# LJacksonPan/RaTrack

Hardware: AMD Instinct MI355X
Metric: radar frame-pairs/sec (backbone forward, eval) at B=64,N=256 per GPU (higher is better)
Workload: dtype f32 (2xfp16 split MFMA: three fp16 products per fp32 product, fp32 accumulate, power-of-two scales per matrix and position); 1 GPU; Track4D.backbone forward, B=64 frame-pairs x N=256 points per GPU, S=512 centroids, eval-mode BN, random-init weights, hipGraph=True, batches in flight=4; global_batch=64, parallelism=replicas x1 (no collective on the forward path)

## Files before the change

### include/rtk_fused.h

```cpp
#ifndef RTK_FUSED_H
#define RTK_FUSED_H

#include "rtk_pointnet2.h"

#ifdef __cplusplus
extern "C" {
#endif

#define RTK_MAX_SRC 4
#define RTK_MAX_LAYERS 4

typedef struct {
    const float *ptr;
    int pitch;
    int channels;
    int per_sample;
} rtk_src_t;

#define RTK_LAYER_SPLIT 0x100
typedef struct {
    const float *w_packed;
    const float *bias;
    int cin16, cout16;
    int act;
// ... 55 lines not shown
                                     int out_pitch, int out_channel_major, rtk_stream_t stream);

RTK_EXPORT int rtk_pack_split_layer(int cout, int cin, const float *w, int transposed, void *image, float *inv_scale,
                                    rtk_stream_t stream);
RTK_EXPORT int rtk_cost_volume_split(int samples, int n1, int n2, const float *xyz1, const float *xyz2,
                                     const int64_t *knn_idx, const float *p1, const float *p2, const float *wd_packed,
                                     const void *split_images, const float *image_scales, const float *bias2,
                                     const float *bias3, const rtk_layer_t *wn, float *out, int out_pitch, rtk_stream_t stream);
RTK_EXPORT int rtk_cost_volume_split_shared(int samples, int n1, int n2, const float *xyz1, const float *xyz2,
                                            const int64_t *knn_idx, const float *p1, const float *p2, const float *wd_packed,
                                            const void *split_images, const float *image_scales, const float *bias2,
                                            const float *bias3, const rtk_layer_t *wn, float *out, int out_pitch, int workgroups,
                                            rtk_stream_t stream);
RTK_EXPORT int rtk_cost_volume_split_gconst(int samples, int n1, int n2, const float *xyz1, const float *xyz2,
                                            const int64_t *knn_idx, const float *p1, const float *p2, const float *wd_packed,
                                            const void *split_images, const float *image_scales, const float *bias2,
                                            const float *bias3, const rtk_layer_t *wn, float *out, int out_pitch, int workgroups,
                                            rtk_stream_t stream);
RTK_EXPORT int rtk_cost_volume_split_term(int samples, int n1, int n2, const float *xyz1, const float *xyz2,
                                          const int64_t *knn_idx, const float *p1, const float *p2, const float *sample_term,
                                          const float *wd_packed, const void *split_images, const float *image_scales,
                                          const float *bias2, const float *bias3, const rtk_layer_t *wn, float *out, int out_pitch,
                                          int workgroups, rtk_stream_t stream);
RTK_EXPORT int rtk_sa_scale_split(int samples, int n, int npoint, int nsample, const float *xyz, const float *new_xyz,
                                  const int *idx, const float *q, int q_pitch, int c1, const float *w1xyz_packed,
                                  const void *split_image, const float *image_scale, const float *bias2, float *out, int out_pitch,
                                  int out_offset, const int *src_nuniq, const int *dst_nuniq, rtk_stream_t stream);
RTK_EXPORT int rtk_sa_scale_split_serial(int samples, int n, int npoint, int nsample, const float *xyz, const float *new_xyz,
                                         const int *idx, const float *q, int q_pitch, int c1, const float *w1xyz_packed,
                                         const void *split_image, const float *image_scale, const float *bias2, float *out,
                                         int out_pitch, int out_offset, const int *src_nuniq, const int *dst_nuniq,
                                         rtk_stream_t stream);
RTK_EXPORT int rtk_split_mlp2(int positions, const float *x, const void *images, const float *image_scales, const float *bias1,
                              const float *bias2, float *y, rtk_stream_t stream);

RTK_EXPORT int rtk_prepare_inputs(int b, int n, const float *pc1, const float *pc2, const float *feature1,
                                  const float *feature2, float *xyz, float *raw, rtk_stream_t stream);

RTK_EXPORT int rtk_fps_centroids(int b, int n, int npoint, const float *xyz, int *idx, float *new_xyz, int *nuniq,
                                 int *tie, const int *n_valid, float *snap, int *first_tie, rtk_stream_t stream);

RTK_EXPORT int rtk_knn_point_masked(int b, int s, int n, int k, const float *query, const float *points, int64_t *idx,
                                    const int *n_valid, rtk_stream_t stream);

RTK_EXPORT int rtk_fps_relevel(int b, int npoint, int levels, const float *xyz1, const int *nuniq1, const int *tie,
                               int *idx, float *new_xyz, int *nuniq, int *tie_work, const int *idx1, const float *snap1,
// ... 115 lines not shown
```

### ratrack_amd/abi.py

```python
import ctypes

import torch

_i, _l, _f, _d, _p = ctypes.c_int, ctypes.c_long, ctypes.c_float, ctypes.c_double, ctypes.c_void_p
_ip, _fp, _pp, P = ctypes.POINTER(_i), ctypes.POINTER(_f), ctypes.POINTER(_p), ctypes.POINTER



class Src(ctypes.Structure):
    _fields_ = [("ptr", _p), ("pitch", _i), ("channels", _i), ("per_sample", _i)]


class Layer(ctypes.Structure):
    _fields_ = [("w_packed", _p), ("bias", _p), ("cin16", _i), ("cout16", _i), ("act", _i), ("inv_scale", _f)]


class Interp(ctypes.Structure):
    _fields_ = [("known_feats", _p), ("pitch", _i), ("channels", _i), ("m", _i), ("idx", _p), ("dist2", _p), ("nuniq", _p)]


class GtermJob(ctypes.Structure):
    _fields_ = [("wt", _p), ("bias", _p), ("out", _p), ("cout", _i), ("s0", _i), ("count", _i), ("out_pitch", _i), ("wt2", _p), ("s2", _i)]


# ... 122 lines not shown
    "rtk_group_points_grad": [_i] * 5 + [_p] * 3 + [_p],
    "rtk_group_points_grad_set": [_i] * 5 + [_p] * 3 + [_p],
    "rtk_three_nn": [_i] * 3 + [_p] * 4 + [_p],
    "rtk_knn": [_i] * 4 + [_p] * 4 + [_p],
    "rtk_three_interpolate": [_i] * 4 + [_p] * 4 + [_p],
    "rtk_three_interpolate_grad": [_i] * 4 + [_p] * 4 + [_p],
    "rtk_three_interpolate_grad_set": [_i] * 4 + [_p] * 4 + [_p],
    "rtk_knn_point": [_i] * 4 + [_p] * 3 + [_p],
    "rtk_pointwise_mlp": [_i, _i, P(Interp), _i, P(Src), _p, _i, P(Layer), _p, _i, _i, _i, _p, _p, _p],
    "rtk_pointwise_mlp_pipelined": [_i, _i, P(Interp), _i, P(Src), _p, _i, P(Layer), _p, _i, _i, _i, _p, _p, _p],
    "rtk_pointwise_mlp_tap": [_i, _i, P(Interp), P(Layer), _p, _i, _p, P(Layer), _i, _p, _i, _p],
    "rtk_pointwise_mlp_tap_pipelined": [_i, _i, P(Interp), P(Layer), _p, _i, _p, P(Layer), _i, _p, _i, _p],
    "rtk_pointwise_mlp_pair": [_i, _i, _i, P(Src), _p, P(Layer), _p, _i, _i, _i, P(Layer), _p, _i, _p],
    "rtk_sa_scale": [_i] * 4 + [_p] * 4 + [_i, _i, _p, _i, P(Layer), _p, _i, _i, _p, _p, _p],
    "rtk_sa_scale_serial": [_i] * 4 + [_p] * 4 + [_i, _i, _p, _i, P(Layer), _p, _i, _i, _p, _p, _p],
    "rtk_cost_volume": [_i] * 3 + [_p] * 6 + [P(Layer), P(Layer), _p, _i, _p],
    "rtk_patch_cost": [_i] * 2 + [_p] * 3 + [_i, P(Layer), _p, _i, _i, _p],
    "rtk_patch_cost_wave16": [_i] * 2 + [_p] * 3 + [_i, P(Layer), _p, _i, _i, _p],
    "rtk_pack_split_layer": [_i, _i, _p, _i, _p, _p, _p],
    "rtk_cost_volume_split": [_i] * 3 + [_p] * 10 + [P(Layer), _p, _i, _p],
    "rtk_cost_volume_split_shared": [_i] * 3 + [_p] * 10 + [P(Layer), _p, _i, _i, _p],
    "rtk_cost_volume_split_gconst": [_i] * 3 + [_p] * 10 + [P(Layer), _p, _i, _i, _p],
    "rtk_cost_volume_split_term": [_i] * 3 + [_p] * 11 + [P(Layer), _p, _i, _i, _p],
    "rtk_sa_scale_split": [_i] * 4 + [_p] * 4 + [_i, _i, _p, _p, _p, _p, _p, _i, _i, _p, _p, _p],
    "rtk_sa_scale_split_serial": [_i] * 4 + [_p] * 4 + [_i, _i, _p, _p, _p, _p, _p, _i, _i, _p, _p, _p],
    "rtk_split_mlp2": [_i, _p, _p, _p, _p, _p, _p, _p],
    "rtk_prepare_inputs": [_i] * 2 + [_p] * 6 + [_p],
    "rtk_fps_centroids": [_i] * 3 + [_p] * 8 + [_p],
    "rtk_knn_point_masked": [_i] * 4 + [_p] * 4 + [_p],
    "rtk_fps_relevel": [_i] * 3 + [_p] * 9 + [_i, _p, _p],
    "rtk_gru_step": [_i] * 3 + [_p] * 8 + [_p],
    "rtk_gru_step_head": [_i] * 3 + [_p] * 11 + [_i, _p],
    "rtk_global_terms": [_i, _i, _p, _i, P(GtermJob), _p, _i, _i, _p],
    "rtk_copy_multi": [_i, P(CopyJob), _p],
    "rtk_to_channel_major": [_i] * 3 + [_p, _i, _i, _p, _i, _i, _p],
    "rtk_ball_query_pair": [_i] * 3 + [_f, _i, _f, _i] + [_p] * 5 + [_p],
    "rtk_three_nn_masked": [_i] * 3 + [_p] * 6 + [_p],
    "rtk_geometry_front": [_i] * 4 + [_p, _p, _i] + [_p] * 13 + [_p, _p, _i, _p],
    "rtk_geometry_tables": [_i] * 3 + [_p] * 3 + [_fp, _ip, _pp, _pp, _pp, _p],
    "rtk_to_channel_major_multi": [_i] * 3 + [_p, _p],
    "rtk_log_sinkhorn": [_i, _i, _p, _f, _i, _p, _p],
    "rtk_dbscan": [_i, _p, _i, _p, _p, _f, _d, _i, _p, _p],
    "rtk_dbscan_batched": [_p, _f, _d, _i, _i, _p, _p, _p, _p, _p, _l, _p],
    "rtk_object_descriptors": [_p, _i, _p, _p, _p, _p, _p, _p],
    "rtk_affinity_pairs": [_i, _i] + [_p] * 7 + [_p],
    "rtk_associate_batched": [_i] * 3 + [_p] * 7 + [_f, _i] + [_p] * 9 + [_p],
# ... 99 lines not shown
```

### ratrack_amd/csrc/fused_split.hip

```cpp
#include "rtk_common.h"
#include "rtk_fused.h"
#include "split_mfma.h"

namespace {

#ifndef SP_NW
#define SP_NW 4
#endif
#ifndef SP_F
#define SP_F 32
#endif
constexpr int CV_F = 32;

__global__ __launch_bounds__(256) void pack_split_kernel(int cout, int cin, const float *__restrict__ w, int transposed, u4v *__restrict__ out,
                                                         float *__restrict__ inv_scale) {
    __shared__ unsigned s_m[4];
    float m = 0.f;
    const f4 *w4 = reinterpret_cast<const f4 *>(w);
    for (int i = threadIdx.x; i < cout * cin / 4; i += 256) {
        const f4 t = w4[i];
        m = __builtin_fmaxf(__builtin_fmaxf(m, __builtin_fabsf(t.x)), __builtin_fabsf(t.y));
        m = __builtin_fmaxf(__builtin_fmaxf(m, __builtin_fabsf(t.z)), __builtin_fabsf(t.w));
    }
    unsigned mb = __float_as_uint(m);
#pragma unroll
    for (int d = 32; d >= 1; d >>= 1) { const unsigned o = __shfl_xor(mb, d, 64); mb = o > mb ? o : mb; }
    if ((threadIdx.x & 63) == 0) s_m[threadIdx.x >> 6] = mb;
    __syncthreads();
    mb = max(max(s_m[0], s_m[1]), max(s_m[2], s_m[3]));
    const LaneScale sc = lane_scale_of(mb);
    if (blockIdx.x == 0 && threadIdx.x == 0) *inv_scale = sc.inv;
    const int VB = cout / 32, slot = blockIdx.x * 256 + threadIdx.x;
    if (slot >= (cin / 16) * VB * 64) return;
    const int lane = slot & 63, v = (slot >> 6) % VB, s = (slot >> 6) / VB, hh = lane >> 5, i = lane & 31;
    const int o = 32 * v + i, c0 = 32 * (s >> 1) + 16 * (s & 1) + 4 * hh;
    f4 x0, x1;
    if (transposed) {
#pragma unroll
        for (int r = 0; r < 4; ++r) { x0[r] = w[(size_t)(c0 + r) * cout + o]; x1[r] = w[(size_t)(c0 + 8 + r) * cout + o]; }
    } else {
        const float *row = w + (size_t)o * cin + c0;
        x0 = *reinterpret_cast<const f4 *>(row); x1 = *reinterpret_cast<const f4 *>(row + 8);
    }
    u4v b[2];
    split2(x0, x1, sc.s, b);
#pragma unroll
    for (int p = 0; p < 2; ++p) out[((size_t)(s * VB + v) * 2 + p) * 64 + lane] = b[p];
}

__device__ __forceinline__ f4 leaky_med4(f4 t, float inf) {
    const f4 u = t * 0.1f;
    return (f4){__builtin_amdgcn_fmed3f(t.x, u.x, inf), __builtin_amdgcn_fmed3f(t.y, u.y, inf), __builtin_amdgcn_fmed3f(t.z, u.z, inf),
                __builtin_amdgcn_fmed3f(t.w, u.w, inf)};
}
__device__ __forceinline__ f4 scale_bias4(f4 a, float c, f4 b) { return __builtin_elementwise_fma(a, (f4){c, c, c, c}, b); }

__global__ __launch_bounds__(64 * SP_NW) __attribute__((amdgpu_waves_per_eu(1, 1)))
void split_mlp2_kernel(int positions, const float *__restrict__ x, const f4 *__restrict__ blob, const float *__restrict__ wsc,
                       const float *__restrict__ bias1, const float *__restrict__ bias2, float *__restrict__ y) {
    const float kinf = rtk_hidden_inf();
    __shared__ __attribute__((aligned(16))) f4 s_w[2 * SP_F * 64];
    const int lane = threadIdx.x & 63, wave = __builtin_amdgcn_readfirstlane(threadIdx.x >> 6), hh = lane >> 5, col = lane & 31;
    constexpr int NF = 2 * SPLIT_NF;
    WStreamA<SP_NW, SP_F, NF> ws;
    ws.start_parts(blob, s_w, wave, lane);
// ... 408 lines not shown
                for (int e = 0; e < 4; ++e) r[q][e] = relu1(w[4 * q + e], kinf) * h[4 * v + q][e];
            const f4 t = row_sum16_transpose4(r[0], r[1], r[2], r[3]);
            if (valid && (j & 3) == 0) *reinterpret_cast<f4 *>(o + 32 * v + 8 * (2 * ((j >> 3) & 1) + ((j >> 2) & 1))) = t;
        };
        out_block(0);
        out_block(1);
        float cn[6] = {0.f, 0.f, 0.f, 0.f, 0.f, 0.f};
        f4 q0n = q0, q1n = q1, s0n = q0, s1n = q1;
        if (more) {
#pragma unroll
            for (int c = 0; c < 3; ++c) { cn[c] = ldc(P.xyz2 + nbn * 3 + c); cn[3 + c] = ldc(P.xyz1 + in_ * 3 + c); }
            q0n = ldc4(P.p1 + in_ * 256 + 4 * hh + 8 * j); q1n = ldc4(P.p1 + in_ * 256 + 4 * hh + 8 * (16 + j));
        }
        if (more && P.st) { s0n = ldc4(P.st + bn * 256 + 4 * hh + 8 * j); s1n = ldc4(P.st + bn * 256 + 4 * hh + 8 * (16 + j)); }
#pragma unroll
        for (int v = 2; v < SPLIT_VB; ++v) out_block(v);
        pt = ptn; valid = validn; i = in_; nb = nbn; q0 = q0n; q1 = q1n;
        if (P.st) { q0 = add4_rn(q0n, s0n); q1 = add4_rn(q1n, s1n); }
        dx = __fsub_rn(cn[0], cn[3]); dy = __fsub_rn(cn[1], cn[4]); dz = __fsub_rn(cn[2], cn[5]);
    }
    ws.finish();
}

struct CvSplitBwdParams {
    CvSplitParams f;
    const float *dout;
    int dout_pitch;
    const float *a3;
    const uint2 *mk1, *mk2;
    float *dz1, *dz2, *dz3, *dq3, *d4, *dp1, *dpd, *dt2, *dbrows;
};

__device__ __forceinline__ f4 leaky_grad_bits4(f4 d, unsigned bits) {
    return (f4){(bits & 1u) ? d.x : 0.1f * d.x, (bits & 2u) ? d.y : 0.1f * d.y, (bits & 4u) ? d.z : 0.1f * d.z, (bits & 8u) ? d.w : 0.1f * d.w};
}

__global__ __launch_bounds__(64 * SP_NW) __attribute__((amdgpu_waves_per_eu(1, 1))) void cost_volume_bwd_split_kernel(const CvSplitBwdParams Q) {
    const float kinf = rtk_hidden_inf();
    __shared__ __attribute__((aligned(16))) f4 s_w[2 * SP_F * 64];
    __shared__ float s_wct[128 * 64];
    const CvSplitParams &P = Q.f;
    const int lane = threadIdx.x & 63, wave = __builtin_amdgcn_readfirstlane(threadIdx.x >> 6), hh = lane >> 5, col = lane & 31, pp = col >> 4,
              j = col & 15;
    const int jq = 2 * ((j >> 3) & 1) + ((j >> 2) & 1);
    for (int e = threadIdx.x; e < 128 * 64; e += 64 * SP_NW) {
        const int l = e & 63, st = e >> 6, o = l & 31, ch = 32 * (st >> 4) + 8 * ((st >> 2) & 3) + 4 * (l >> 5) + (st & 3);
// ... 478 lines not shown
        float *o = P.out + (long)c * P.out_pitch + P.out_offset + 4 * hh + 8 * qo;
        if constexpr (NS == 32) {
            f4 t[4];
#pragma unroll
            for (int q = 0; q < 4; ++q) t[q] = wave_max_pair16(m[0][q], m[1][q], kinf);
            const f4 r = relu_med4(row_max16_transpose4(t[0], t[1], t[2], t[3]), kinf);
            if (valid && (col & 3) == 0) *reinterpret_cast<f4 *>(o + 32 * ((col >> 4) & 1)) = r;
        } else {
#pragma unroll
            for (int v = 0; v < 2; ++v) {
                const f4 r = relu_med4(row_max16_transpose4(m[v][0], m[v][1], m[v][2], m[v][3]), kinf);
                if (valid && (col & 3) == 0) *reinterpret_cast<f4 *>(o + 32 * v) = r;
            }
        }
    }
}

}

extern "C" int rtk_pack_split_layer(int cout, int cin, const float *w, int transposed, void *image, float *inv_scale, rtk_stream_t stream) {
    RTK_REQUIRE(cout > 0 && cin > 0 && cout % 32 == 0 && cin % 32 == 0 && w && image && inv_scale, "pack_split_layer: bad arguments");
    RTK_REQUIRE((long)cout * cin <= (1L << 22), "pack_split_layer: more than 2^22 weights (every workgroup scans the matrix for its scale)");
    const int slots = (cin / 16) * (cout / 32) * 64;
    pack_split_kernel<<<(slots + 255) / 256, 256, 0, (hipStream_t)stream>>>(cout, cin, w, transposed, (u4v *)image, inv_scale);
    RTK_CHECK_LAUNCH("pack_split_layer");
    return RTK_OK;
}

extern "C" int rtk_split_mlp2(int positions, const float *x, const void *images, const float *image_scales, const float *bias1,
                              const float *bias2, float *y, rtk_stream_t stream) {
    RTK_REQUIRE(positions > 0 && x && images && image_scales && bias1 && bias2 && y, "split_mlp2: bad arguments");
    const int tiles = (positions + 32 * SP_NW - 1) / (32 * SP_NW);
    split_mlp2_kernel<<<tiles < 256 ? tiles : 256, 64 * SP_NW, 0, (hipStream_t)stream>>>(positions, x, (const f4 *)images, image_scales, bias1, bias2, y);
    RTK_CHECK_LAUNCH("split_mlp2");
    return RTK_OK;
}

static int cv_split_fill(const char *who, CvSplitParams &P, int samples, int n1, int n2, const float *xyz1, const float *xyz2,
                         const int64_t *knn_idx, const void *split_images, const float *image_scales, const rtk_layer_t *wn, dim3 &grid) {
    RTK_REQUIRE(samples > 0 && samples <= 65535 && n1 > 0 && n2 >= 16 && xyz1 && xyz2 && knn_idx && split_images && image_scales,
                "%s: bad arguments", who);
    RTK_REQUIRE(wn && wn[0].w_packed && wn[1].w_packed && wn[2].w_packed && wn[1].bias && wn[2].bias && wn[1].cin16 == 1 &&
                wn[1].cout16 == 1 && wn[2].cin16 == 1 && wn[2].cout16 == 16, "%s: bad WeightNet layers", who);
    P.samples = samples; P.n1 = n1; P.n2 = n2;
    P.xyz1 = xyz1; P.xyz2 = xyz2; P.knn = knn_idx;
    P.blob = reinterpret_cast<const f4 *>(split_images);
    P.wsc = image_scales;
    P.wn.wa = wn[0].w_packed; P.wn.wb = wn[1].w_packed; P.wn.wc = wn[2].w_packed; P.wn.bb = wn[1].bias; P.wn.bc = wn[2].bias;
    P.p1 = P.p2 = P.st = P.wd = P.bias2 = P.bias3 = nullptr;
    P.out = nullptr; P.out_pitch = 0; P.sv1 = P.sv2 = P.sv3 = nullptr; P.mk1 = P.mk2 = nullptr; P.amax = nullptr;
    const int groups = (n1 + 2 * SP_NW - 1) / (2 * SP_NW);
    int gx = 256 / samples;
    if (gx < 1) gx = 1;
    if (gx > groups) gx = groups;
    grid = rtk_xcd_grid(samples, gx, P.gx);
    return RTK_OK;
}

static int cu_count() {
    int dev = 0, n = 0;
    if (hipGetDevice(&dev) != hipSuccess || hipDeviceGetAttribute(&n, hipDeviceAttributeMultiprocessorCount, dev) != hipSuccess || n < 8) return 256;
    return n;
}

static int cv_split_forward(const char *who, int samples, int n1, int n2, const float *xyz1, const float *xyz2, const int64_t *knn_idx,
                            const float *p1, const float *p2, const float *wd_packed, const void *split_images, const float *image_scales,
                            const float *bias2, const float *bias3, const rtk_layer_t *wn, float *out, int out_pitch, float *a1, float *a2,
                            float *a3, void *mask1, void *mask2, float *amax, int workgroups, rtk_stream_t stream,
                            const float *sample_term = nullptr, bool global_consts = false) {
    CvSplitParams P;
    dim3 grid;
    if (cv_split_fill(who, P, samples, n1, n2, xyz1, xyz2, knn_idx, split_images, image_scales, wn, grid) != RTK_OK) return RTK_ERR_INVALID;
    RTK_REQUIRE(p1 && p2 && wd_packed && bias2 && bias3 && out, "%s: bad arguments", who);
    RTK_REQUIRE((double)samples * n2 <= 4194304.0, "%s: more than 2^22 rows in p2 (32-bit byte offsets of the row requests): split the batch", who);
    RTK_REQUIRE(out_pitch % 4 == 0 && out_pitch >= 256, "%s: bad out_pitch", who);
    const bool save = a1 != nullptr;
    RTK_REQUIRE(!save || ((double)samples * n1 * 16.0 * 1024.0 < 4294967296.0), "%s: more than 4 GiB per saved activation (32-bit row "
                "offsets): split the batch", who);
    P.p1 = p1; P.p2 = p2; P.st = sample_term; P.wd = wd_packed; P.bias2 = bias2; P.bias3 = bias3; P.out = out; P.out_pitch = out_pitch;
    P.sv1 = a1; P.sv2 = a2; P.sv3 = a3; P.mk1 = (uint2 *)mask1; P.mk2 = (uint2 *)mask2; P.amax = amax;
    if (samples % 8 == 0) {
        const int tiles_x = (samples / 8) * ((n1 + 2 * SP_NW - 1) / (2 * SP_NW));
        int per_xcd = (workgroups > 0 ? workgroups : cu_count()) / 8;
        if (per_xcd < 1) per_xcd = 1;
        if (per_xcd > tiles_x) per_xcd = tiles_x;
        P.gx = 8 * per_xcd;
        grid = dim3(P.gx);
    }
    if (save) cost_volume_split_kernel<true><<<grid, 64 * SP_NW, 0, (hipStream_t)stream>>>(P);
    else if (global_consts) cost_volume_split_kernel<false, false><<<grid, 64 * SP_NW, 0, (hipStream_t)stream>>>(P);
    else cost_volume_split_kernel<false><<<grid, 64 * SP_NW, 0, (hipStream_t)stream>>>(P);
    RTK_CHECK_LAUNCH(who);
    return RTK_OK;
}

extern "C" int rtk_cost_volume_split(int samples, int n1, int n2, const float *xyz1, const float *xyz2, const int64_t *knn_idx,
                                     const float *p1, const float *p2, const float *wd_packed, const void *split_images,
                                     const float *image_scales, const float *bias2, const float *bias3, const rtk_layer_t *wn, float *out,
                                     int out_pitch, rtk_stream_t stream) {
    return cv_split_forward("cost_volume_split", samples, n1, n2, xyz1, xyz2, knn_idx, p1, p2, wd_packed, split_images, image_scales, bias2, bias3,
                            wn, out, out_pitch, nullptr, nullptr, nullptr, nullptr, nullptr, nullptr, 0, stream);
}

extern "C" int rtk_cost_volume_split_shared(int samples, int n1, int n2, const float *xyz1, const float *xyz2, const int64_t *knn_idx,
                                            const float *p1, const float *p2, const float *wd_packed, const void *split_images,
                                            const float *image_scales, const float *bias2, const float *bias3, const rtk_layer_t *wn,
                                            float *out, int out_pitch, int workgroups, rtk_stream_t stream) {
    RTK_REQUIRE(workgroups >= 0, "cost_volume_split_shared: workgroups = %d", workgroups);
    return cv_split_forward("cost_volume_split_shared", samples, n1, n2, xyz1, xyz2, knn_idx, p1, p2, wd_packed, split_images, image_scales,
                            bias2, bias3, wn, out, out_pitch, nullptr, nullptr, nullptr, nullptr, nullptr, nullptr, workgroups, stream);
}

extern "C" int rtk_cost_volume_split_gconst(int samples, int n1, int n2, const float *xyz1, const float *xyz2, const int64_t *knn_idx,
                                            const float *p1, const float *p2, const float *wd_packed, const void *split_images,
                                            const float *image_scales, const float *bias2, const float *bias3, const rtk_layer_t *wn,
                                            float *out, int out_pitch, int workgroups, rtk_stream_t stream) {
    RTK_REQUIRE(workgroups >= 0, "cost_volume_split_gconst: workgroups = %d", workgroups);
    return cv_split_forward("cost_volume_split_gconst", samples, n1, n2, xyz1, xyz2, knn_idx, p1, p2, wd_packed, split_images, image_scales,
                            bias2, bias3, wn, out, out_pitch, nullptr, nullptr, nullptr, nullptr, nullptr, nullptr, workgroups, stream, nullptr, true);
}

extern "C" int rtk_cost_volume_split_term(int samples, int n1, int n2, const float *xyz1, const float *xyz2, const int64_t *knn_idx,
                                          const float *p1, const float *p2, const float *sample_term, const float *wd_packed,
                                          const void *split_images, const float *image_scales, const float *bias2, const float *bias3,
                                          const rtk_layer_t *wn, float *out, int out_pitch, int workgroups, rtk_stream_t stream) {
    RTK_REQUIRE(workgroups >= 0 && sample_term, "cost_volume_split_term: workgroups = %d, sample_term = %p", workgroups, (const void *)sample_term);
    return cv_split_forward("cost_volume_split_term", samples, n1, n2, xyz1, xyz2, knn_idx, p1, p2, wd_packed, split_images, image_scales,
                            bias2, bias3, wn, out, out_pitch, nullptr, nullptr, nullptr, nullptr, nullptr, nullptr, workgroups, stream, sample_term);
}

extern "C" int rtk_cost_volume_split_train(int samples, int n1, int n2, const float *xyz1, const float *xyz2, const int64_t *knn_idx,
                                           const float *p1, const float *p2, const float *wd_packed, const void *split_images,
                                           const float *image_scales, const float *bias2, const float *bias3, const rtk_layer_t *wn,
                                           float *out, int out_pitch, float *a1, float *a2, float *a3, void *mask1, void *mask2,
                                           float *act_amax, rtk_stream_t stream) {
    RTK_REQUIRE(a1 && a2 && a3 && mask1 && mask2, "cost_volume_split_train: null activation buffer");
    return cv_split_forward("cost_volume_split_train", samples, n1, n2, xyz1, xyz2, knn_idx, p1, p2, wd_packed, split_images, image_scales,
                            bias2, bias3, wn, out, out_pitch, a1, a2, a3, mask1, mask2, act_amax, 0, stream);
}

extern "C" int rtk_cost_volume_bwd_split(int samples, int n1, int n2, const float *xyz1, const float *xyz2, const int64_t *knn_idx,
                                         const void *split_images_t, const float *image_scales_t, const rtk_layer_t *wn, const float *dout,
                                         int dout_pitch,
                                         const float *a3, const void *mask1, const void *mask2, float *dz1, float *dz2, float *dz3,
                                         float *dq3, float *d4, float *dp1, float *dpd, float *dt2, float *dbias_rows,
                                         float *dz_amax, rtk_stream_t stream) {
    CvSplitBwdParams Q;
    dim3 grid;
    if (cv_split_fill("cost_volume_bwd_split", Q.f, samples, n1, n2, xyz1, xyz2, knn_idx, split_images_t, image_scales_t, wn, grid) != RTK_OK)
        return RTK_ERR_INVALID;
    RTK_REQUIRE(dout && mask1 && mask2 && a3 && dz1 && dz2 && dz3 && dq3 && d4 && dp1 && dpd && dt2, "cost_volume_bwd_split: bad arguments");
// ... 64 lines not shown
```

### ratrack_amd/fused.py

```python
import ctypes
import os
import types

import torch

from . import _lib
from . import pointnet2_hip as _native
from .abi import CopyJob as _CopyJob, GtermJob as _GtJob, Interp as _Interp, Layer as _Layer, Src as _Src, ptr as _ptr, stream as _stream

ACT_NONE, ACT_RELU, ACT_LEAKY, ACT_SIGMOID = 0, 1, 2, 3


def copy_multi(pairs):
    for i in range(0, len(pairs), 8):
        part = pairs[i:i + 8]
        jobs = (_CopyJob * len(part))()
        for j, (d, s_) in enumerate(part):
            assert d.is_contiguous() and s_.is_contiguous() and d.shape == s_.shape and d.dtype == s_.dtype and d.device == s_.device
            jobs[j].src, jobs[j].dst, jobs[j].bytes = s_.data_ptr(), d.data_ptr(), d.numel() * d.element_size()
        _lib.call("rtk_copy_multi", len(part), jobs, _stream())


def ceil16(c):
    return (c + 15) // 16 * 16
# ... 497 lines not shown
        if self.side is not None:
            ev = torch.cuda.Event()
            ev.record(self.side)
            self.events[key] = ev

    def wait(self, key):
        ev = self.events.get(key)
        if ev is not None:
            torch.cuda.current_stream().wait_event(ev)

    def head(self, count):
        g = object.__new__(Geometry)
        g.n, g.samples, g.npoint = self.n, count, self.npoint
        g.xyz = [x[:count] for x in self.xyz]
        g.ball = [[b[:count] for b in row] for row in self.ball]
        g.nuniq = [c[:count] for c in self.nuniq]
        g.fps_idx, g.tie = [i[:count] for i in self.fps_idx], self.tie[:count]
        g.events, g.knn, g.side = self.events, self.knn, self.side
        g.nn = {k: (d2[:count], idx[:count], m) for k, (d2, idx, m) in self.nn.items()}
        return g


CV_SPLIT_MAX_ROWS = 1 << 22


def cv_shared_workgroups(samples, n1, dev):
    cus = torch.cuda.get_device_properties(dev).multi_processor_count
    if samples % 8 or cus % 8:
        return 0
    tiles = (samples // 8) * ((n1 + 7) // 8)
    lo, hi = max(1, cus // 16), max(1, cus // 8 * 3 // 4)
    balance = lambda w: tiles / (w * -(-tiles // w))
    ok = [w for w in range(hi, lo - 1, -1) if balance(w) >= 0.95]
    w = ok[0] if ok else max(range(lo, hi + 1), key=balance)
    return 8 * min(w, tiles)


SA_ENTRIES = ("rtk_sa_scale", "rtk_sa_scale_split")
SA_ENTRIES_SERIAL = ("rtk_sa_scale_serial", "rtk_sa_scale_split_serial")


def sa_scale(geo, W, lvl, s, q, qcol, out, out_offset):
    sc = W.scales[lvl][s]
    qptr, qpitch = _colptr(q, qcol)
    optr, opitch = _colptr(out)
    src, dst = geo.xyz[lvl], geo.xyz[lvl + 1]
# ... 75 lines not shown
        self.enc = _PNHeadWeights(sd, "pn_head.", dev)
        self.dec = _PNHeadWeights(sd, "fd_layer.mse.", dev)
        z = lambda n: torch.zeros(n, dtype=torch.float64, device=sd["bin_score"].device)
        self.enc_q1 = Chain([(self.enc.wq1, z(32), ACT_NONE)], dev)
        self.enc_q1_w = self.enc.wq1.float().to(dev).contiguous()
        w0 = sd["fc_layer.mlp_convs.0.weight"].double().reshape(256, 515)
        b0 = sd["fc_layer.mlp_convs.0.bias"].double()
        self.p1_loc = Chain([(w0[:, 0:128], z(256), ACT_NONE)], dev)
        self.p2_loc = Chain([(w0[:, 256:384], z(256), ACT_NONE)], dev)
        tr = lambda w: w.float().t().contiguous().to(dev)
        self.p1_glob_wt, self.p1_glob_b = tr(w0[:, 128:256]), b0.float().to(dev).contiguous()
        self.p2_glob_wt = tr(w0[:, 384:512])
        self.cv_wd = offset_image(torch.cat([w0[:, 512:515], z(256)[:, None]], 1), dev)
        self.cv_layers = Chain([(sd["fc_layer.mlp_convs.%d.weight" % i].double().reshape(256, 256),
                                 sd["fc_layer.mlp_convs.%d.bias" % i].double(), ACT_LEAKY) for i in (1, 2)], dev)
        self.cv_split = bool(split)
        w23 = [sd["fc_layer.mlp_convs.%d.weight" % i].double().reshape(256, 256).float().to(dev).contiguous() for i in (1, 2)]
        self.cv_bias23 = torch.stack([sd["fc_layer.mlp_convs.%d.bias" % i].double().float() for i in (1, 2)]).to(dev).contiguous()
        self.cv_images = torch.empty(2 * SPLIT_IMAGE_256, dtype=torch.int16, device=dev)
        self.cv_scales = torch.empty(2, dtype=torch.float32, device=dev)
        for l, w in enumerate(w23):
            _lib.call("rtk_pack_split_layer", 256, 256, w.data_ptr(), 0, self.cv_images[l * SPLIT_IMAGE_256:].data_ptr(),
                      self.cv_scales[l:].data_ptr(), _stream())
        torch.cuda.current_stream().synchronize()
        self.wn1 = _WeightNet(sd, "fc_layer.weightnet1", dev)
        self.wn2 = _WeightNet(sd, "fc_layer.weightnet2", dev)
        def predictor(prefix, first_cols):
            layers = []
            for i in range(3):
                w, b = fold_bn(sd["%s.sf_mlp.%d.0.weight" % (prefix, i)], "%s.sf_mlp.%d.1" % (prefix, i), sd)
                layers.append([w, b, ACT_RELU])
            return layers
        cp = predictor("fd_layer.cp", None)
        wl, bl = sd["fd_layer.cp.linear.weight"].double(), sd["fd_layer.cp.linear.bias"].double()
        wc2 = sd["fd_layer.cp.conv2.weight"].double().reshape(3, 32)
        cp.append([wl @ wc2, bl, ACT_SIGMOID])
        self.cls_head = Chain([tuple(x) for x in cp], dev)
        fp = predictor("fd_layer.fp", None)
        w_first = fp[0][0]
        self.flow_glob_wt, self.flow_glob_b = tr(w_first[:, 128:256]), fp[0][1].float().to(dev).contiguous()
        fp[0] = [w_first[:, 0:128], z(128), ACT_RELU]
        fp.append([sd["fd_layer.fp.conv2.weight"].double().reshape(3, 32), z(3), ACT_NONE])
        self.flow_head = Chain([tuple(x) for x in fp], dev)
        wq = self.dec.wq1
        wq_pad = torch.zeros(32, 16, dtype=torch.float64, device=wq.device)
        wq_pad[:, :2] = wq[:, 0:2]
# ... 70 lines not shown
            q1d = pointwise(B * N, N, dsrc, self.dec_q1, new(B * N, 32), sample_bias=sbq)
        prop, gfeat = run_pnhead(self.dec, geo.head(B), q1d, gmax=gmax[2 * B:])
        if h is None:
            h = torch.zeros(5, B, 128, device=dev, dtype=torch.float32)
        gout, h_out, sbf = self._gru_step(gfeat, h)
        flow = torch.empty(B, 3, N, dtype=torch.float32, device=dev)
        pointwise(B * N, N, [(prop, 128, False)], self.flow_head, flow, out_channels=3, sample_bias=sbf, channel_major=True)
        f12 = feat12.view(2 * B, N, 256).permute(0, 2, 1)
        pc1_features, pc2_features = f12[:B], f12[B:]
        cor_cm = cor.view(B, N, 256).permute(0, 2, 1)
        prop_cm = prop.view(B, N, 128).permute(0, 2, 1)
        return flow, h_out, cls, cor_cm, pc1_features, pc2_features, prop_cm

    def _cost_volume(self, B, N, x1, x2, knn1, p1, p2, cor1, sample_term=None):
        assert sample_term is None or self.cv_split
        if _TRACE is not None:
            _TRACE.append(("cost_volume", B * N * 16, 3 * 256 + 2 * 256 * 256 + (3 * 8 + 8 * 8 + 8 * 256) + 256))
        if self.cv_split:
            step = B if B * N <= CV_SPLIT_MAX_ROWS else max(1, CV_SPLIT_MAX_ROWS // N)
            for b0 in range(0, B, step):
                nb = min(step, B - b0)
                wgs = cv_shared_workgroups(nb, N, x1.device) if self.cv_shared else 0
                r0 = b0 * N
                if sample_term is not None:
                    _lib.call("rtk_cost_volume_split_term", nb, N, N, x1[b0:].data_ptr(), x2[b0:].data_ptr(), knn1[b0:].data_ptr(),
                              p1[r0:].data_ptr(), p2[r0:].data_ptr(), sample_term[b0:].data_ptr(), self.cv_wd.data_ptr(),
                              self.cv_images.data_ptr(), self.cv_scales.data_ptr(), self.cv_bias23[0].data_ptr(), self.cv_bias23[1].data_ptr(),
                              self.wn1.arr, cor1[r0:].data_ptr(), 256, wgs, _stream())
                    continue
                _lib.call("rtk_cost_volume_split_shared", nb, N, N, x1[b0:].data_ptr(), x2[b0:].data_ptr(), knn1[b0:].data_ptr(), p1[r0:].data_ptr(),
                          p2[r0:].data_ptr(), self.cv_wd.data_ptr(), self.cv_images.data_ptr(), self.cv_scales.data_ptr(),
                          self.cv_bias23[0].data_ptr(), self.cv_bias23[1].data_ptr(), self.wn1.arr, cor1[r0:].data_ptr(), 256, wgs, _stream())
            return
        _lib.call("rtk_cost_volume", B, N, N, x1.data_ptr(), x2.data_ptr(), knn1.data_ptr(), p1.data_ptr(), p2.data_ptr(),
                  self.cv_wd.data_ptr(), self.cv_layers.arr, self.wn1.arr, cor1.data_ptr(), 256, _stream())

    def _gru_step(self, x, h):
        L, B, H = h.shape
        if _TRACE is not None:
            _TRACE.append(("gru", B * L, 2 * 3 * H * H))
            _TRACE.append(("global_terms", B, H * self.flow_glob_wt.shape[1]))
        h_out = torch.empty_like(h)
        y = torch.empty(B, H, dtype=torch.float32, device=h.device)
        sbf = torch.empty(B, self.flow_glob_wt.shape[1], dtype=torch.float32, device=h.device)
        h = h.contiguous()
        _lib.call("rtk_gru_step_head", B, L, H, x.data_ptr(), h.data_ptr(), self.gru_wih.data_ptr(), self.gru_whh.data_ptr(),
                  self.gru_bih.data_ptr(), self.gru_bhh.data_ptr(), h_out.data_ptr(), y.data_ptr(), self.flow_glob_wt.data_ptr(),
                  self.flow_glob_b.data_ptr(), sbf.data_ptr(), sbf.shape[1], _stream())
        return y, h_out, sbf

    def clone(self):
        import copy
        e = copy.copy(self)
        e.side, e._last_cv, e.kernel_events, e.kernel_token = None, None, None, None
# ... 149 lines not shown
```

Before: 123,700 frame-pairs/s.

## Add 16x16 MFMA tile variant of split cost-volume kernel, enabled by default

Adds a new cost-volume kernel that runs the two 256x256 split-fp16 layers with 16-wide MFMA tiles (one 16-neighbour point per wave, 8 waves per workgroup), plus a matching weight-packing layout. It also adds a bank-conflict-free LDS staging layout for the neighbour feature rows and a separate constant block. The intent is better MFMA efficiency and data reuse in the dominant cost-volume stage than the 32-wide tile gives. The costs are higher register and LDS pressure, two waves per EU, and a second packed weight copy. Scales still come from the 32-tile pack.

```diff
diff --git a/include/rtk_fused.h b/include/rtk_fused.h
--- a/include/rtk_fused.h
+++ b/include/rtk_fused.h
@@ -101,6 +101,18 @@
                                           const float *wd_packed, const void *split_images, const float *image_scales,
                                           const float *bias2, const float *bias3, const rtk_layer_t *wn, float *out, int out_pitch,
                                           int workgroups, rtk_stream_t stream);
+RTK_EXPORT int rtk_pack_split_layer16(int cout, int cin, const float *w, int transposed, void *image, float *inv_scale,
+                                      rtk_stream_t stream);
+RTK_EXPORT int rtk_cost_volume_split16_shared(int samples, int n1, int n2, const float *xyz1, const float *xyz2,
+                                              const int64_t *knn_idx, const float *p1, const float *p2, const float *wd_packed,
+                                              const void *split_images16, const float *image_scales, const float *bias2,
+                                              const float *bias3, const rtk_layer_t *wn, float *out, int out_pitch, int workgroups,
+                                              rtk_stream_t stream);
+RTK_EXPORT int rtk_cost_volume_split16_term(int samples, int n1, int n2, const float *xyz1, const float *xyz2,
+                                            const int64_t *knn_idx, const float *p1, const float *p2, const float *sample_term,
+                                            const float *wd_packed, const void *split_images16, const float *image_scales,
+                                            const float *bias2, const float *bias3, const rtk_layer_t *wn, float *out, int out_pitch,
+                                            int workgroups, rtk_stream_t stream);
 RTK_EXPORT int rtk_sa_scale_split(int samples, int n, int npoint, int nsample, const float *xyz, const float *new_xyz,
                                   const int *idx, const float *q, int q_pitch, int c1, const float *w1xyz_packed,
                                   const void *split_image, const float *image_scale, const float *bias2, float *out, int out_pitch,
diff --git a/ratrack_amd/abi.py b/ratrack_amd/abi.py
--- a/ratrack_amd/abi.py
+++ b/ratrack_amd/abi.py
@@ -168,6 +168,9 @@
     "rtk_cost_volume_split_shared": [_i] * 3 + [_p] * 10 + [P(Layer), _p, _i, _i, _p],
     "rtk_cost_volume_split_gconst": [_i] * 3 + [_p] * 10 + [P(Layer), _p, _i, _i, _p],
     "rtk_cost_volume_split_term": [_i] * 3 + [_p] * 11 + [P(Layer), _p, _i, _i, _p],
+    "rtk_pack_split_layer16": [_i, _i, _p, _i, _p, _p, _p],
+    "rtk_cost_volume_split16_shared": [_i] * 3 + [_p] * 10 + [P(Layer), _p, _i, _i, _p],
+    "rtk_cost_volume_split16_term": [_i] * 3 + [_p] * 11 + [P(Layer), _p, _i, _i, _p],
     "rtk_sa_scale_split": [_i] * 4 + [_p] * 4 + [_i, _i, _p, _p, _p, _p, _p, _i, _i, _p, _p, _p],
     "rtk_sa_scale_split_serial": [_i] * 4 + [_p] * 4 + [_i, _i, _p, _p, _p, _p, _p, _i, _i, _p, _p, _p],
     "rtk_split_mlp2": [_i, _p, _p, _p, _p, _p, _p, _p],
diff --git a/ratrack_amd/csrc/fused_split.hip b/ratrack_amd/csrc/fused_split.hip
--- a/ratrack_amd/csrc/fused_split.hip
+++ b/ratrack_amd/csrc/fused_split.hip
@@ -12,6 +12,7 @@
 #endif
 constexpr int CV_F = 32;
 
+template <bool TILE16>
 __global__ __launch_bounds__(256) void pack_split_kernel(int cout, int cin, const float *__restrict__ w, int transposed, u4v *__restrict__ out,
                                                          float *__restrict__ inv_scale) {
     __shared__ unsigned s_m[4];
@@ -30,17 +31,18 @@
     mb = max(max(s_m[0], s_m[1]), max(s_m[2], s_m[3]));
     const LaneScale sc = lane_scale_of(mb);
     if (blockIdx.x == 0 && threadIdx.x == 0) *inv_scale = sc.inv;
-    const int VB = cout / 32, slot = blockIdx.x * 256 + threadIdx.x;
-    if (slot >= (cin / 16) * VB * 64) return;
+    const int VB = cout / (TILE16 ? 16 : 32), slot = blockIdx.x * 256 + threadIdx.x;
+    if (slot >= (cin / (TILE16 ? 32 : 16)) * VB * 64) return;
     const int lane = slot & 63, v = (slot >> 6) % VB, s = (slot >> 6) / VB, hh = lane >> 5, i = lane & 31;
-    const int o = 32 * v + i, c0 = 32 * (s >> 1) + 16 * (s & 1) + 4 * hh;
+    constexpr int C1 = TILE16 ? 16 : 8;
+    const int o = TILE16 ? 16 * v + (lane & 15) : 32 * v + i, c0 = TILE16 ? 32 * s + 4 * (lane >> 4) : 32 * (s >> 1) + 16 * (s & 1) + 4 * hh;
     f4 x0, x1;
     if (transposed) {
 #pragma unroll
-        for (int r = 0; r < 4; ++r) { x0[r] = w[(size_t)(c0 + r) * cout + o]; x1[r] = w[(size_t)(c0 + 8 + r) * cout + o]; }
+        for (int r = 0; r < 4; ++r) { x0[r] = w[(size_t)(c0 + r) * cout + o]; x1[r] = w[(size_t)(c0 + C1 + r) * cout + o]; }
     } else {
         const float *row = w + (size_t)o * cin + c0;
-        x0 = *reinterpret_cast<const f4 *>(row); x1 = *reinterpret_cast<const f4 *>(row + 8);
+        x0 = *reinterpret_cast<const f4 *>(row); x1 = *reinterpret_cast<const f4 *>(row + C1);
     }
     u4v b[2];
     split2(x0, x1, sc.s, b);
@@ -495,6 +497,253 @@
     ws.finish();
 }
 
+constexpr int CV16_NW = 8;
+constexpr int CV16_V = 16;
+constexpr int CV16_KS = 8;
+constexpr int CV16_NF = CV16_KS * CV16_V * 2;
+constexpr int CV16_ROWS_F4 = 16 * 32;
+constexpr int cv16_rows_slot(int pos, int chunk) { return pos * 32 + (chunk ^ pos); }
+constexpr bool cv16_rows_conflict_free() {
+    constexpr int served[2][16] = {{0, 1, 2, 3, 12, 13, 14, 15, 20, 21, 22, 23, 24, 25, 26, 27}, {4, 5, 6, 7, 8, 9, 10, 11, 16, 17, 18, 19, 28, 29, 30, 31}};
+    for (int u = 0; u < 8; ++u)
+        for (int half = 0; half < 2; ++half)
+            for (int grp = 0; grp < 2; ++grp) {
+                unsigned seen = 0u;
+                for (int k = 0; k < 16; ++k) {
+                    const int lane = 32 * half + served[grp][k], g = lane >> 4, j = lane & 15;
+                    const unsigned bankgroup = 1u << (cv16_rows_slot(j, 4 * u + g) & 15);
+                    if (seen & bankgroup) return false;
+                    seen |= bankgroup;
+                }
+            }
+    return true;
+}
+static_assert(cv16_rows_conflict_free(), "a ds_read_b128 of the staged rows must touch 16 different bank groups per lane group");
+static_assert(cv16_rows_slot(15, 31) < CV16_ROWS_F4, "a position's chunks stay inside its own 512 bytes");
+
+struct CvConsts16 {
+    float wd[CV16_V * 64];
+    float wc[CV16_V * 2 * 64];
+    float bc[256], bias2[256], bias3[256];
+    float hid[128];
+};
+static_assert(sizeof(CvConsts16) == 15 * 1024 + 512, "4 + 8 + 3 KiB + the hidden layers");
+__device__ __forceinline__ void cv16_consts_fill(CvConsts16 &C, const float *wd, const WnSplit &W, const float *bias2, const float *bias3, int t) {
+    if (t < 256) *reinterpret_cast<f4 *>(C.wd + 4 * t) = ldc4(wd + 4 * t);
+    else if (t < 256 + 192) {
+        const int which = (t - 256) >> 6, l = t & 63;
+        *reinterpret_cast<f4 *>((which == 0 ? C.bc : which == 1 ? C.bias2 : C.bias3) + 4 * l) = ldc4((which == 0 ? W.bc : which == 1 ? bias2 : bias3) + 4 * l);
+    }
+#pragma unroll
+    for (int n = 0; n < 4; ++n) {
+        const int e = 512 * n + t, v = e >> 7, s = (e >> 6) & 1, l = e & 63, k = 2 * (l >> 4) + s;
+        C.wc[e] = ldc(W.wc + ((v * 64 + 16 * (k >> 2) + (l & 15)) * 4 + (k & 3)));
+    }
+    if (t < 104) {
+        const int u = t < 32 ? 0 : t - 32, o = u >> 3, c = u & 7;
+        C.hid[t] = ldc(t < 32 ? W.wa + 16 * (t >> 3) + (t & 7) : t < 96 ? W.wb + (16 * (c >> 2) + o) * 4 + (c & 3) : W.bb + (t - 96));
+    }
+}
+
+__device__ __forceinline__ void cv16_wn_hidden(const CvConsts16 &C, float dx, float dy, float dz, float (&t2)[8]) {
+    float t1[8];
+#pragma unroll
+    for (int o = 0; o < 8; ++o) {
+        float a = __fmaf_rn(C.hid[o], dx, 0.f);
+        a = __fmaf_rn(C.hid[8 + o], dy, a);
+        a = __fmaf_rn(C.hid[16 + o], dz, a);
+        t1[o] = fmaxf(__fadd_rn(a, C.hid[24 + o]), 0.f);
+    }
+    __builtin_amdgcn_sched_barrier(0);
+#pragma unroll
+    for (int o = 0; o < 8; ++o) {
+        float a = C.hid[96 + o];
+#pragma unroll
+        for (int c = 0; c < 8; ++c) a = __fmaf_rn(C.hid[32 + 8 * o + c], t1[c], a);
+        t2[o] = fmaxf(a, 0.f);
+        asm volatile("" : "+v"(t2[o]));
+        if (o % 4 == 3) __builtin_amdgcn_sched_barrier(0);
+    }
+}
+
+template <int HALF>
+__device__ __forceinline__ void cv16_rows_request(const float *p2, int nbrow, f4 *rows, int lane) {
+    asm volatile("s_waitcnt lgkmcnt(0)" ::: "memory");
+    CvRowsRequest(p2, rows, nbrow, HALF, lane).all(std::make_integer_sequence<int, 8>{});
+}
+template <int HALF>
+__device__ __forceinline__ void cv16_rows_read(const f4 *rows, int j, int g, f4 (&h)[CV16_V]) {
+#pragma unroll
+    for (int u = 0; u < 8; ++u) h[8 * HALF + u] = rows[j * 32 + ((4 * u + g) ^ j)];
+}
+template <int U0>
+__device__ __forceinline__ void cv16_layer1_blocks(const CvConsts16 &C, const f4 q, float bop, int lane, float kinf, f4 (&h)[CV16_V]) {
+    auto block = [&](auto uc) {
+        constexpr int u = decltype(uc)::value;
+        h[u] = leaky_med4(mfma4(C.wd[u * 64 + lane], bop, add_row_bcast<u>(q, h[u])), kinf);
+    };
+    block(std::integral_constant<int, U0>{}); block(std::integral_constant<int, U0 + 1>{});
+    block(std::integral_constant<int, U0 + 2>{}); block(std::integral_constant<int, U0 + 3>{});
+    block(std::integral_constant<int, U0 + 4>{}); block(std::integral_constant<int, U0 + 5>{});
+    block(std::integral_constant<int, U0 + 6>{}); block(std::integral_constant<int, U0 + 7>{});
+}
+
+template <int FBASE, int GI, class WS, int F, bool ZERO>
+struct Split16Step {
+    static constexpr int GV = CV16_V / 2, NG = CV16_KS * GV;
+    template <int GJ, int PART>
+    static __device__ __forceinline__ void load_part(WS &ws, f4 (&dst)[SPLIT_GF]) {
+        constexpr int f0 = FBASE + GJ * SPLIT_GF;
+        if constexpr (PART == 0) {
+            if constexpr (f0 % F == 0 && f0 != 0) ws.sync();
+            if constexpr ((f0 % F) / SPLIT_GF < split_issue_groups(F)) ws.template issue_part<(f0 % F) / SPLIT_GF, split_issue_groups(F)>();
+        }
+        dst[2 * PART] = ws.template frag_async<(f0 + 2 * PART) % F>();
+        dst[2 * PART + 1] = ws.template frag_async<(f0 + 2 * PART + 1) % F>();
+    }
+    static __device__ __forceinline__ void run(WS &ws, const f4 (&h)[CV16_V], float scale, f4 (&acc)[CV16_V], f4 (&a)[2][SPLIT_GF], u4v (&b)[2][2]) {
+        constexpr int up = GI / GV, v0 = (GI % GV) * 2;
+        static_assert(F % SPLIT_GF == 0, "a group step reads four consecutive fragments of one chunk");
+        lds_wait<0>(a[GI & 1]);
+        const f4(&c)[SPLIT_GF] = a[GI & 1];
+        const u4v(&B)[2] = b[up & 1];
+        f4 z0, z1;
+        if constexpr (ZERO && up == 0) z0 = z1 = f4_zero();
+        else { z0 = acc[v0]; z1 = acc[v0 + 1]; }
+        acc[v0] = mfma16_h(__builtin_bit_cast(u4v, c[1]), B[0], z0);
+        acc[v0 + 1] = mfma16_h(__builtin_bit_cast(u4v, c[3]), B[0], z1);
+        if constexpr (GI + 1 < NG) load_part<GI + 1, 0>(ws, a[(GI + 1) & 1]);
+        __builtin_amdgcn_sched_barrier(0);
+        acc[v0] = mfma16_h(__builtin_bit_cast(u4v, c[0]), B[1], acc[v0]);
+        acc[v0 + 1] = mfma16_h(__builtin_bit_cast(u4v, c[2]), B[1], acc[v0 + 1]);
+        if constexpr (GI + 1 < NG) load_part<GI + 1, 1>(ws, a[(GI + 1) & 1]);
+        __builtin_amdgcn_sched_barrier(0);
+        if constexpr (up + 1 < CV16_KS && GI % GV < 4) split2_word_of<GI % GV>(h[2 * (up + 1)], h[2 * (up + 1) + 1], scale, b[(up + 1) & 1]);
+        acc[v0] = mfma16_h(__builtin_bit_cast(u4v, c[0]), B[0], acc[v0]);
+        acc[v0 + 1] = mfma16_h(__builtin_bit_cast(u4v, c[2]), B[0], acc[v0 + 1]);
+        __builtin_amdgcn_sched_barrier(0);
+    }
+};
+template <int FBASE, class WS, int F, bool ZERO, int... GI>
+__device__ __forceinline__ void split16_layer_impl(WS &ws, const f4 (&h)[CV16_V], float scale, f4 (&acc)[CV16_V], std::integer_sequence<int, GI...>) {
+    f4 a[2][SPLIT_GF];
+    u4v b[2][2];
+    Split16Step<FBASE, 0, WS, F, ZERO>::template load_part<0, 0>(ws, a[0]);
+    Split16Step<FBASE, 0, WS, F, ZERO>::template load_part<0, 1>(ws, a[0]);
+    split2(h[0], h[1], scale, b[0]);
+    __builtin_amdgcn_sched_barrier(0);
+    (Split16Step<FBASE, GI, WS, F, ZERO>::run(ws, h, scale, acc, a, b), ...);
+}
+template <int FBASE, int NW, int F, int NF>
+__device__ __forceinline__ void split16_layer(WStreamA<NW, F, NF> &ws, const f4 (&h)[CV16_V], float scale, f4 (&acc)[CV16_V]) {
+    split16_layer_impl<FBASE, WStreamA<NW, F, NF>, F, true>(ws, h, scale, acc, std::make_integer_sequence<int, CV16_KS * (CV16_V / 2)>{});
+}
+
+__global__ __launch_bounds__(64 * CV16_NW) __attribute__((amdgpu_waves_per_eu(2, 2)))
+void cost_volume_split_kernel16(const CvSplitParams P) {
+    const float kinf = rtk_hidden_inf();
+    __shared__ __attribute__((aligned(16))) f4 s_w[2 * CV_F * 64];
+    __shared__ __attribute__((aligned(16))) f4 s_rows[CV16_NW * CV16_ROWS_F4];
+    __shared__ __attribute__((aligned(16))) CvConsts16 s_c;
+    const int lane = threadIdx.x & 63, wave = __builtin_amdgcn_readfirstlane(threadIdx.x >> 6), g = lane >> 4, j = lane & 15;
+    f4 *rows = s_rows + wave * CV16_ROWS_F4;
+    constexpr int PPW = CV16_NW;
+    const int groups = (P.n1 + PPW - 1) / PPW;
+    const bool flat = P.gx > 0;
+    const int xcd = blockIdx.x & 7, t0 = flat ? (int)(blockIdx.x >> 3) : (int)blockIdx.x, tstep = flat ? P.gx >> 3 : (int)gridDim.x;
+    const int ntiles = flat ? (P.samples >> 3) * groups : groups;
+    auto locate = [&](int t, int &b_, int &G_) {
+        if (flat) { const int sk = t / groups; b_ = sk * 8 + xcd; G_ = t - sk * groups; }
+        else { b_ = blockIdx.y; G_ = t; }
+    };
+    int b, bx;
+    locate(t0 < ntiles ? t0 : 0, b, bx);
+    cv16_consts_fill(s_c, P.wd, P.wn, P.bias2, P.bias3, (int)threadIdx.x);
+    WStreamA<CV16_NW, CV_F, 2 * CV16_NF> ws;
+    ws.start_parts(P.blob, s_w, wave, lane);
+    const float wi2 = ldc(P.wsc), wi3 = ldc(P.wsc + 1);
+    bool valid = bx * PPW + wave < P.n1;
+    long i = (long)b * P.n1 + (valid ? bx * PPW + wave : P.n1 - 1);
+    long nb = 0;
+    float dx = 0.f, dy = 0.f, dz = 0.f;
+    f4 q = {0.f, 0.f, 0.f, 0.f};
+    if (t0 < ntiles) {
+        nb = (long)b * P.n2 + (long)P.knn[i * 16 + j];
+        cv16_rows_request<0>(P.p2, (int)nb, rows, lane);
+        q = ldc4(P.p1 + i * 256 + 16 * j + 4 * g);
+        if (P.st) q = add4_rn(q, ldc4(P.st + b * 256 + 16 * j + 4 * g));
+        dx = __fsub_rn(P.xyz2[nb * 3], P.xyz1[i * 3]); dy = __fsub_rn(P.xyz2[nb * 3 + 1], P.xyz1[i * 3 + 1]);
+        dz = __fsub_rn(P.xyz2[nb * 3 + 2], P.xyz1[i * 3 + 2]);
+    }
+    for (int t = t0; t < ntiles; t += tstep) {
+        asm volatile("" ::: "memory");
+        int lv = lane;
+        asm volatile("" : "+v"(lv));
+        const int jv = lv & 15, gv = lv >> 4;
+        const bool more = t + tstep < ntiles;
+        int bn, Gn;
+        locate(more ? t + tstep : t, bn, Gn);
+        const bool validn = Gn * PPW + wave < P.n1;
+        const long in_ = (long)bn * P.n1 + (validn ? Gn * PPW + wave : P.n1 - 1);
+        long knn_next = 0;
+        if (more) knn_next = (long)P.knn[in_ * 16 + j];
+        f4 h[CV16_V];
+        float t2[8];
+        {
+            const float bop = g == 0 ? dx : g == 1 ? dy : g == 2 ? dz : 0.f;
+            cv16_rows_read<0>(rows, jv, gv, h);
+            cv16_rows_request<1>(P.p2, (int)nb, rows, lv);
+            cv16_layer1_blocks<0>(s_c, q, bop, lane, kinf, h);
+            cv16_wn_hidden(s_c, dx, dy, dz, t2);
+            __builtin_amdgcn_sched_barrier(0);
+            cv16_rows_read<1>(rows, jv, gv, h);
+            cv16_layer1_blocks<8>(s_c, q, bop, lane, kinf, h);
+        }
+        const long nbn = (long)bn * P.n2 + knn_next;
+        if (more) cv16_rows_request<0>(P.p2, (int)nbn, rows, lv);
+        f4 acc[CV16_V];
+        LaneScale sc = lane_scale16(h);
+        split16_layer<0>(ws, h, sc.s, acc);
+        float c = sc.inv * wi2;
+#pragma unroll
+        for (int v = 0; v < CV16_V; ++v) h[v] = leaky_med4(scale_bias4(acc[v], c, *reinterpret_cast<const f4 *>(s_c.bias2 + 16 * v + 4 * g)), kinf);
+        sc = lane_scale16(h);
+        split16_layer<CV16_NF>(ws, h, sc.s, acc);
+        ws.sync();
+        c = sc.inv * wi3;
+#pragma unroll
+        for (int v = 0; v < CV16_V; ++v) h[v] = leaky_med4(scale_bias4(acc[v], c, *reinterpret_cast<const f4 *>(s_c.bias3 + 16 * v + 4 * g)), kinf);
+        float cn[6] = {0.f, 0.f, 0.f, 0.f, 0.f, 0.f};
+        f4 qn = q, sn = q;
+        if (more) {
+#pragma unroll
+            for (int k = 0; k < 3; ++k) { cn[k] = ldc(P.xyz2 + nbn * 3 + k); cn[3 + k] = ldc(P.xyz1 + in_ * 3 + k); }
+            qn = ldc4(P.p1 + in_ * 256 + 16 * j + 4 * g);
+        }
+        if (more && P.st) sn = ldc4(P.st + bn * 256 + 16 * j + 4 * g);
+        const float tb0 = g == 0 ? t2[0] : g == 1 ? t2[2] : g == 2 ? t2[4] : t2[6], tb1 = g == 0 ? t2[1] : g == 1 ? t2[3] : g == 2 ? t2[5] : t2[7];
+        float *o = P.out + i * P.out_pitch + 4 * g + 16 * (2 * ((j >> 3) & 1) + ((j >> 2) & 1));
+#pragma unroll
+        for (int m = 0; m < CV16_V / 4; ++m) {
+            f4 r[4];
+#pragma unroll
+            for (int e = 0; e < 4; ++e) {
+                const int v = 4 * m + e;
+                f4 w = *reinterpret_cast<const f4 *>(s_c.bc + 16 * v + 4 * g);
+                w = mfma4(s_c.wc[(2 * v) * 64 + lane], tb0, w);
+                w = mfma4(s_c.wc[(2 * v + 1) * 64 + lane], tb1, w);
+                r[e] = relu_med4(w, kinf) * h[v];
+            }
+            const f4 s = row_sum16_transpose4(r[0], r[1], r[2], r[3]);
+            if (valid && (j & 3) == 0) *reinterpret_cast<f4 *>(o + 64 * m) = s;
+        }
+        valid = validn; i = in_; nb = nbn; q = qn;
+        if (P.st) q = add4_rn(qn, sn);
+        dx = __fsub_rn(cn[0], cn[3]); dy = __fsub_rn(cn[1], cn[4]); dz = __fsub_rn(cn[2], cn[5]);
+    }
+    ws.finish();
+}
+
 struct CvSplitBwdParams {
     CvSplitParams f;
     const float *dout;
@@ -1019,8 +1268,17 @@
     RTK_REQUIRE(cout > 0 && cin > 0 && cout % 32 == 0 && cin % 32 == 0 && w && image && inv_scale, "pack_split_layer: bad arguments");
     RTK_REQUIRE((long)cout * cin <= (1L << 22), "pack_split_layer: more than 2^22 weights (every workgroup scans the matrix for its scale)");
     const int slots = (cin / 16) * (cout / 32) * 64;
-    pack_split_kernel<<<(slots + 255) / 256, 256, 0, (hipStream_t)stream>>>(cout, cin, w, transposed, (u4v *)image, inv_scale);
+    pack_split_kernel<false><<<(slots + 255) / 256, 256, 0, (hipStream_t)stream>>>(cout, cin, w, transposed, (u4v *)image, inv_scale);
     RTK_CHECK_LAUNCH("pack_split_layer");
+    return RTK_OK;
+}
+
+extern "C" int rtk_pack_split_layer16(int cout, int cin, const float *w, int transposed, void *image, float *inv_scale, rtk_stream_t stream) {
+    RTK_REQUIRE(cout > 0 && cin > 0 && cout % 32 == 0 && cin % 32 == 0 && w && image && inv_scale, "pack_split_layer16: bad arguments");
+    RTK_REQUIRE((long)cout * cin <= (1L << 22), "pack_split_layer16: more than 2^22 weights (every workgroup scans the matrix for its scale)");
+    const int slots = (cin / 32) * (cout / 16) * 64;
+    pack_split_kernel<true><<<(slots + 255) / 256, 256, 0, (hipStream_t)stream>>>(cout, cin, w, transposed, (u4v *)image, inv_scale);
+    RTK_CHECK_LAUNCH("pack_split_layer16");
     return RTK_OK;
 }
 
@@ -1064,7 +1322,7 @@
                             const float *p1, const float *p2, const float *wd_packed, const void *split_images, const float *image_scales,
                             const float *bias2, const float *bias3, const rtk_layer_t *wn, float *out, int out_pitch, float *a1, float *a2,
                             float *a3, void *mask1, void *mask2, float *amax, int workgroups, rtk_stream_t stream,
-                            const float *sample_term = nullptr, bool global_consts = false) {
+                            const float *sample_term = nullptr, bool global_consts = false, bool tile16 = false) {
     CvSplitParams P;
     dim3 grid;
     if (cv_split_fill(who, P, samples, n1, n2, xyz1, xyz2, knn_idx, split_images, image_scales, wn, grid) != RTK_OK) return RTK_ERR_INVALID;
@@ -1084,7 +1342,9 @@
         P.gx = 8 * per_xcd;
         grid = dim3(P.gx);
     }
-    if (save) cost_volume_split_kernel<true><<<grid, 64 * SP_NW, 0, (hipStream_t)stream>>>(P);
+    static_assert(2 * SP_NW == CV16_NW, "both tiles take eight points per workgroup iteration: one grid rule");
+    if (tile16) cost_volume_split_kernel16<<<grid, 64 * CV16_NW, 0, (hipStream_t)stream>>>(P);
+    else if (save) cost_volume_split_kernel<true><<<grid, 64 * SP_NW, 0, (hipStream_t)stream>>>(P);
     else if (global_consts) cost_volume_split_kernel<false, false><<<grid, 64 * SP_NW, 0, (hipStream_t)stream>>>(P);
     else cost_volume_split_kernel<false><<<grid, 64 * SP_NW, 0, (hipStream_t)stream>>>(P);
     RTK_CHECK_LAUNCH(who);
@@ -1124,6 +1384,26 @@
     RTK_REQUIRE(workgroups >= 0 && sample_term, "cost_volume_split_term: workgroups = %d, sample_term = %p", workgroups, (const void *)sample_term);
     return cv_split_forward("cost_volume_split_term", samples, n1, n2, xyz1, xyz2, knn_idx, p1, p2, wd_packed, split_images, image_scales,
                             bias2, bias3, wn, out, out_pitch, nullptr, nullptr, nullptr, nullptr, nullptr, nullptr, workgroups, stream, sample_term);
+}
+
+extern "C" int rtk_cost_volume_split16_shared(int samples, int n1, int n2, const float *xyz1, const float *xyz2, const int64_t *knn_idx,
+                                              const float *p1, const float *p2, const float *wd_packed, const void *split_images16,
+                                              const float *image_scales, const float *bias2, const float *bias3, const rtk_layer_t *wn,
+                                              float *out, int out_pitch, int workgroups, rtk_stream_t stream) {
+    RTK_REQUIRE(workgroups >= 0, "cost_volume_split16_shared: workgroups = %d", workgroups);
+    return cv_split_forward("cost_volume_split16_shared", samples, n1, n2, xyz1, xyz2, knn_idx, p1, p2, wd_packed, split_images16, image_scales,
+                            bias2, bias3, wn, out, out_pitch, nullptr, nullptr, nullptr, nullptr, nullptr, nullptr, workgroups, stream, nullptr, false,
+                            true);
+}
+
+extern "C" int rtk_cost_volume_split16_term(int samples, int n1, int n2, const float *xyz1, const float *xyz2, const int64_t *knn_idx,
+                                            const float *p1, const float *p2, const float *sample_term, const float *wd_packed,
+                                            const void *split_images16, const float *image_scales, const float *bias2, const float *bias3,
+                                            const rtk_layer_t *wn, float *out, int out_pitch, int workgroups, rtk_stream_t stream) {
+    RTK_REQUIRE(workgroups >= 0 && sample_term, "cost_volume_split16_term: workgroups = %d, sample_term = %p", workgroups, (const void *)sample_term);
+    return cv_split_forward("cost_volume_split16_term", samples, n1, n2, xyz1, xyz2, knn_idx, p1, p2, wd_packed, split_images16, image_scales,
+                            bias2, bias3, wn, out, out_pitch, nullptr, nullptr, nullptr, nullptr, nullptr, nullptr, workgroups, stream, sample_term,
+                            false, true);
 }
 
 extern "C" int rtk_cost_volume_split_train(int samples, int n1, int n2, const float *xyz1, const float *xyz2, const int64_t *knn_idx,
diff --git a/ratrack_amd/fused.py b/ratrack_amd/fused.py
--- a/ratrack_amd/fused.py
+++ b/ratrack_amd/fused.py
@@ -543,6 +543,7 @@
 
 
 CV_SPLIT_MAX_ROWS = 1 << 22
+CV_TILE16 = os.environ.get("RTK_CV_TILE16", "1") == "1"
 
 
 def cv_shared_workgroups(samples, n1, dev):
@@ -664,6 +665,11 @@
         for l, w in enumerate(w23):
             _lib.call("rtk_pack_split_layer", 256, 256, w.data_ptr(), 0, self.cv_images[l * SPLIT_IMAGE_256:].data_ptr(),
                       self.cv_scales[l:].data_ptr(), _stream())
+        self.cv_images16 = torch.empty(2 * SPLIT_IMAGE_256, dtype=torch.int16, device=dev)
+        scales16 = torch.empty(2, dtype=torch.float32, device=dev)
+        for l, w in enumerate(w23):
+            _lib.call("rtk_pack_split_layer16", 256, 256, w.data_ptr(), 0, self.cv_images16[l * SPLIT_IMAGE_256:].data_ptr(),
+                      scales16[l:].data_ptr(), _stream())
         torch.cuda.current_stream().synchronize()
         self.wn1 = _WeightNet(sd, "fc_layer.weightnet1", dev)
         self.wn2 = _WeightNet(sd, "fc_layer.weightnet2", dev)
@@ -780,14 +786,16 @@
                 nb = min(step, B - b0)
                 wgs = cv_shared_workgroups(nb, N, x1.device) if self.cv_shared else 0
                 r0 = b0 * N
+                images = self.cv_images16 if CV_TILE16 else self.cv_images
                 if sample_term is not None:
-                    _lib.call("rtk_cost_volume_split_term", nb, N, N, x1[b0:].data_ptr(), x2[b0:].data_ptr(), knn1[b0:].data_ptr(),
+                    _lib.call("rtk_cost_volume_split16_term" if CV_TILE16 else "rtk_cost_volume_split_term", nb, N, N, x1[b0:].data_ptr(), x2[b0:].data_ptr(), knn1[b0:].data_ptr(),
                               p1[r0:].data_ptr(), p2[r0:].data_ptr(), sample_term[b0:].data_ptr(), self.cv_wd.data_ptr(),
-                              self.cv_images.data_ptr(), self.cv_scales.data_ptr(), self.cv_bias23[0].data_ptr(), self.cv_bias23[1].data_ptr(),
+                              images.data_ptr(), self.cv_scales.data_ptr(), self.cv_bias23[0].data_ptr(), self.cv_bias23[1].data_ptr(),
                               self.wn1.arr, cor1[r0:].data_ptr(), 256, wgs, _stream())
                     continue
-                _lib.call("rtk_cost_volume_split_shared", nb, N, N, x1[b0:].data_ptr(), x2[b0:].data_ptr(), knn1[b0:].data_ptr(), p1[r0:].data_ptr(),
-                          p2[r0:].data_ptr(), self.cv_wd.data_ptr(), self.cv_images.data_ptr(), self.cv_scales.data_ptr(),
+                _lib.call("rtk_cost_volume_split16_shared" if CV_TILE16 else "rtk_cost_volume_split_shared", nb, N, N, x1[b0:].data_ptr(),
+                          x2[b0:].data_ptr(), knn1[b0:].data_ptr(), p1[r0:].data_ptr(),
+                          p2[r0:].data_ptr(), self.cv_wd.data_ptr(), images.data_ptr(), self.cv_scales.data_ptr(),
                           self.cv_bias23[0].data_ptr(), self.cv_bias23[1].data_ptr(), self.wn1.arr, cor1[r0:].data_ptr(), 256, wgs, _stream())
             return
         _lib.call("rtk_cost_volume", B, N, N, x1.data_ptr(), x2.data_ptr(), knn1.data_ptr(), p1.data_ptr(), p2.data_ptr(),
```

Result: faster. 126,300 frame-pairs/s (median of 6 runs) (+2.1%).
